# run-house/kubetorch

Measured on NVIDIA H100. Metric: parallel_map_arg_plus_result_GBps, higher is better.
Workload: dtype f32

## Files before the change

kubetorch_b200/csrc/ktb_mlp.cu:

```cuda
#include "ktb_common.cuh"

#include <cuda.h>
#include <algorithm>
#include <atomic>
#include <climits>
#include <cmath>
#include <mutex>

namespace ktb {

constexpr int kMlpBlockM = 128;
constexpr int kMlpBlockK = 64;
constexpr int kMlpWgmmaK = 16;
constexpr int kMlpStages = 4;
constexpr int kMlpConsumers = 256;
constexpr int kMlpThreads = kMlpConsumers + 32;
int g_mlp_chunk_rows = 16896;

__device__ __forceinline__ void tma_load_2d(void* smem_dst, const CUtensorMap* map, int c0, int c1, uint64_t* bar) {
  asm volatile(
      "cp.async.bulk.tensor.2d.shared::cluster.global.mbarrier::complete_tx::bytes [%0], [%1, {%3, %4}], [%2];" ::
          "r"(smem_u32(smem_dst)),
      "l"(map), "r"(smem_u32(bar)), "r"(c0), "r"(c1)
      : "memory");
}
__device__ __forceinline__ void prefetch_tensormap(const CUtensorMap* map) {
  asm volatile("prefetch.tensormap [%0];" ::"l"(map) : "memory");
}
__device__ __forceinline__ void mbar_arrive(uint64_t* bar) {
  asm volatile("mbarrier.arrive.shared::cta.b64 _, [%0];" ::"r"(smem_u32(bar)) : "memory");
}
__device__ __forceinline__ void wgmma_fence() { asm volatile("wgmma.fence.sync.aligned;" ::: "memory"); }
__device__ __forceinline__ void wgmma_commit() { asm volatile("wgmma.commit_group.sync.aligned;" ::: "memory"); }
__device__ __forceinline__ void wgmma_wait_all() { asm volatile("wgmma.wait_group.sync.aligned 0;" ::: "memory"); }

__device__ __forceinline__ uint64_t make_smem_desc_sw128(const void* smem_tile) {
  const uint32_t addr = smem_u32(smem_tile);
  uint64_t d = 0;
  d |= (uint64_t)((addr & 0x3FFFFu) >> 4);
  d |= (uint64_t)1 << 16;
  d |= (uint64_t)(1024u >> 4) << 32;
  d |= (uint64_t)1 << 62;
  return d;
}

template <int N>
struct Wgmma;
template <>
struct Wgmma<256> {
  __device__ __forceinline__ static void mma(float (&d)[128], uint64_t adesc, uint64_t bdesc, uint32_t scale_d) {
    asm volatile(
        "{\n"
        ".reg .pred p;\n"
        "setp.ne.b32 p, %130, 0;\n"
        "wgmma.mma_async.sync.aligned.m64n256k16.f32.bf16.bf16 "
        "{%0,%1,%2,%3,%4,%5,%6,%7,%8,%9,%10,%11,%12,%13,%14,%15,%16,%17,%18,%19,%20,%21,%22,%23,%24,%25,%26,%27,%28,%29,%30,%31,%32,%33,%34,%35,%36,%37,%38,%39,%40,%41,%42,%43,%44,%45,%46,%47,%48,%49,%50,%51,%52,%53,%54,%55,%56,%57,%58,%59,%60,%61,%62,%63,%64,%65,%66,%67,%68,%69,%70,%71,%72,%73,%74,%75,%76,%77,%78,%79,%80,%81,%82,%83,%84,%85,%86,%87,%88,%89,%90,%91,%92,%93,%94,%95,%96,%97,%98,%99,%100,%101,%102,%103,%104,%105,%106,%107,%108,%109,%110,%111,%112,%113,%114,%115,%116,%117,%118,%119,%120,%121,%122,%123,%124,%125,%126,%127}, "
        "%128, %129, p, 1, 1, 0, 0;\n"
        "}\n"
        : "+f"(d[0]), "+f"(d[1]), "+f"(d[2]), "+f"(d[3]), "+f"(d[4]), "+f"(d[5]), "+f"(d[6]), "+f"(d[7]), "+f"(d[8]), "+f"(d[9]), "+f"(d[10]), "+f"(d[11]), "+f"(d[12]), "+f"(d[13]), "+f"(d[14]), "+f"(d[15]), "+f"(d[16]), "+f"(d[17]), "+f"(d[18]), "+f"(d[19]), "+f"(d[20]), "+f"(d[21]), "+f"(d[22]), "+f"(d[23]), "+f"(d[24]), "+f"(d[25]), "+f"(d[26]), "+f"(d[27]), "+f"(d[28]), "+f"(d[29]), "+f"(d[30]), "+f"(d[31]), "+f"(d[32]), "+f"(d[33]), "+f"(d[34]), "+f"(d[35]), "+f"(d[36]), "+f"(d[37]), "+f"(d[38]), "+f"(d[39]), "+f"(d[40]), "+f"(d[41]), "+f"(d[42]), "+f"(d[43]), "+f"(d[44]), "+f"(d[45]), "+f"(d[46]), "+f"(d[47]), "+f"(d[48]), "+f"(d[49]), "+f"(d[50]), "+f"(d[51]), "+f"(d[52]), "+f"(d[53]), "+f"(d[54]), "+f"(d[55]), "+f"(d[56]), "+f"(d[57]), "+f"(d[58]), "+f"(d[59]), "+f"(d[60]), "+f"(d[61]), "+f"(d[62]), "+f"(d[63]), "+f"(d[64]), "+f"(d[65]), "+f"(d[66]), "+f"(d[67]), "+f"(d[68]), "+f"(d[69]), "+f"(d[70]), "+f"(d[71]), "+f"(d[72]), "+f"(d[73]), "+f"(d[74]), "+f"(d[75]), "+f"(d[76]), "+f"(d[77]), "+f"(d[78]), "+f"(d[79]), "+f"(d[80]), "+f"(d[81]), "+f"(d[82]), "+f"(d[83]), "+f"(d[84]), "+f"(d[85]), "+f"(d[86]), "+f"(d[87]), "+f"(d[88]), "+f"(d[89]), "+f"(d[90]), "+f"(d[91]), "+f"(d[92]), "+f"(d[93]), "+f"(d[94]), "+f"(d[95]), "+f"(d[96]), "+f"(d[97]), "+f"(d[98]), "+f"(d[99]), "+f"(d[100]), "+f"(d[101]), "+f"(d[102]), "+f"(d[103]), "+f"(d[104]), "+f"(d[105]), "+f"(d[106]), "+f"(d[107]), "+f"(d[108]), "+f"(d[109]), "+f"(d[110]), "+f"(d[111]), "+f"(d[112]), "+f"(d[113]), "+f"(d[114]), "+f"(d[115]), "+f"(d[116]), "+f"(d[117]), "+f"(d[118]), "+f"(d[119]), "+f"(d[120]), "+f"(d[121]), "+f"(d[122]), "+f"(d[123]), "+f"(d[124]), "+f"(d[125]), "+f"(d[126]), "+f"(d[127])
        : "l"(adesc), "l"(bdesc), "r"(scale_d));
  }
};

template <>
struct Wgmma<128> {
  __device__ __forceinline__ static void mma(float (&d)[64], uint64_t adesc, uint64_t bdesc, uint32_t scale_d) {
    asm volatile(
        "{\n"
        ".reg .pred p;\n"
        "setp.ne.b32 p, %66, 0;\n"
        "wgmma.mma_async.sync.aligned.m64n128k16.f32.bf16.bf16 "
        "{%0,%1,%2,%3,%4,%5,%6,%7,%8,%9,%10,%11,%12,%13,%14,%15,%16,%17,%18,%19,%20,%21,%22,%23,%24,%25,%26,%27,%28,%29,%30,%31,%32,%33,%34,%35,%36,%37,%38,%39,%40,%41,%42,%43,%44,%45,%46,%47,%48,%49,%50,%51,%52,%53,%54,%55,%56,%57,%58,%59,%60,%61,%62,%63}, "
        "%64, %65, p, 1, 1, 0, 0;\n"
        "}\n"
        : "+f"(d[0]), "+f"(d[1]), "+f"(d[2]), "+f"(d[3]), "+f"(d[4]), "+f"(d[5]), "+f"(d[6]), "+f"(d[7]), "+f"(d[8]), "+f"(d[9]), "+f"(d[10]), "+f"(d[11]), "+f"(d[12]), "+f"(d[13]), "+f"(d[14]), "+f"(d[15]), "+f"(d[16]), "+f"(d[17]), "+f"(d[18]), "+f"(d[19]), "+f"(d[20]), "+f"(d[21]), "+f"(d[22]), "+f"(d[23]), "+f"(d[24]), "+f"(d[25]), "+f"(d[26]), "+f"(d[27]), "+f"(d[28]), "+f"(d[29]), "+f"(d[30]), "+f"(d[31]), "+f"(d[32]), "+f"(d[33]), "+f"(d[34]), "+f"(d[35]), "+f"(d[36]), "+f"(d[37]), "+f"(d[38]), "+f"(d[39]), "+f"(d[40]), "+f"(d[41]), "+f"(d[42]), "+f"(d[43]), "+f"(d[44]), "+f"(d[45]), "+f"(d[46]), "+f"(d[47]), "+f"(d[48]), "+f"(d[49]), "+f"(d[50]), "+f"(d[51]), "+f"(d[52]), "+f"(d[53]), "+f"(d[54]), "+f"(d[55]), "+f"(d[56]), "+f"(d[57]), "+f"(d[58]), "+f"(d[59]), "+f"(d[60]), "+f"(d[61]), "+f"(d[62]), "+f"(d[63])
        : "l"(adesc), "l"(bdesc), "r"(scale_d));
  }
};

template <>
struct Wgmma<64> {
  __device__ __forceinline__ static void mma(float (&d)[32], uint64_t adesc, uint64_t bdesc, uint32_t scale_d) {
    asm volatile(
        "{\n"
        ".reg .pred p;\n"
        "setp.ne.b32 p, %34, 0;\n"
        "wgmma.mma_async.sync.aligned.m64n64k16.f32.bf16.bf16 "
        "{%0,%1,%2,%3,%4,%5,%6,%7,%8,%9,%10,%11,%12,%13,%14,%15,%16,%17,%18,%19,%20,%21,%22,%23,%24,%25,%26,%27,%28,%29,%30,%31}, "
        "%32, %33, p, 1, 1, 0, 0;\n"
        "}\n"
        : "+f"(d[0]), "+f"(d[1]), "+f"(d[2]), "+f"(d[3]), "+f"(d[4]), "+f"(d[5]), "+f"(d[6]), "+f"(d[7]), "+f"(d[8]), "+f"(d[9]), "+f"(d[10]), "+f"(d[11]), "+f"(d[12]), "+f"(d[13]), "+f"(d[14]), "+f"(d[15]), "+f"(d[16]), "+f"(d[17]), "+f"(d[18]), "+f"(d[19]), "+f"(d[20]), "+f"(d[21]), "+f"(d[22]), "+f"(d[23]), "+f"(d[24]), "+f"(d[25]), "+f"(d[26]), "+f"(d[27]), "+f"(d[28]), "+f"(d[29]), "+f"(d[30]), "+f"(d[31])
        : "l"(adesc), "l"(bdesc), "r"(scale_d));
  }
};
template <int BLOCK_N, int STAGES>
struct MlpSmem {
  static constexpr int kABytes = kMlpBlockM * kMlpBlockK * 2;
  static constexpr int kBBytes = BLOCK_N * kMlpBlockK * 2;
  static constexpr int kStageBytes = kABytes + kBBytes;
  static constexpr int kBarrierOff = STAGES * kStageBytes;
  static constexpr int kTotal = kBarrierOff + 2 * STAGES * 8 + 1024 ;
};

template <int BLOCK_N, int STAGES>
__device__ __forceinline__ bool mlp_tile_mainloop(const CUtensorMap* map_a, const CUtensorMap* map_b, int K, int m0,
                                                  int n0, float (&acc)[BLOCK_N / 2]) {
  using S = MlpSmem<BLOCK_N, STAGES>;
  extern __shared__ uint8_t smem_raw[];
  uint8_t* smem = reinterpret_cast<uint8_t*>((reinterpret_cast<uintptr_t>(smem_raw) + 1023) & ~(uintptr_t)1023);
  uint64_t* full = reinterpret_cast<uint64_t*>(smem + S::kBarrierOff);
  uint64_t* empty = full + STAGES;

  const int warp = threadIdx.x >> 5;
  const int lane = threadIdx.x & 31;
  const int num_kb = K / kMlpBlockK;

  if (threadIdx.x == 0) {
#pragma unroll
    for (int s = 0; s < STAGES; ++s) {
      mbar_init(&full[s], 1);
      mbar_init(&empty[s], kMlpConsumers);
    }
    fence_barrier_init();
  }
  __syncthreads();

  if (warp == kMlpConsumers / 32) {
    if (lane == 0) {
      prefetch_tensormap(map_a);
      prefetch_tensormap(map_b);
      for (int kb = 0; kb < num_kb; ++kb) {
        const int s = kb % STAGES;
        mbar_wait(&empty[s], ((kb / STAGES) & 1) ^ 1);
        uint8_t* a_dst = smem + (size_t)s * S::kStageBytes;
        mbar_expect_tx(&full[s], S::kStageBytes);
        tma_load_2d(a_dst, map_a, kb * kMlpBlockK, m0, &full[s]);
        tma_load_2d(a_dst + S::kABytes, map_b, kb * kMlpBlockK, n0, &full[s]);
      }
    }
    return false;
  }

  const int wg = warp >> 2;
#pragma unroll
  for (int i = 0; i < BLOCK_N / 2; ++i) acc[i] = 0.f;
  for (int kb = 0; kb < num_kb; ++kb) {
    const int s = kb % STAGES;
    mbar_wait(&full[s], (kb / STAGES) & 1);
    const uint8_t* a_src = smem + (size_t)s * S::kStageBytes + wg * 64 * 128;
    const uint64_t adesc = make_smem_desc_sw128(a_src);
    const uint64_t bdesc = make_smem_desc_sw128(smem + (size_t)s * S::kStageBytes + S::kABytes);
    wgmma_fence();
#pragma unroll
    for (int k = 0; k < kMlpBlockK / kMlpWgmmaK; ++k) {
      Wgmma<BLOCK_N>::mma(acc, adesc + (uint64_t)(2 * k), bdesc + (uint64_t)(2 * k), (uint32_t)((kb | k) != 0));
    }
    wgmma_commit();
    wgmma_wait_all();
    mbar_arrive(&empty[s]);
  }
  return true;
}

__device__ __forceinline__ bool argmax_before(float v, int col, float best, int best_col) {
  const bool v_nan = v != v, best_nan = best != best;
  if (v_nan || best_nan) return v_nan && (!best_nan || col < best_col);
  return v > best || (v == best && col < best_col);
}

__device__ __forceinline__ void layer_pair(float a0, float a1, float a2, float a3, const __nv_bfloat16* bias, int col,
                                           int n_valid, int relu, __nv_bfloat162& y0, __nv_bfloat162& y1) {
  float v[4] = {a0, a1, a2, a3};
  if (bias != nullptr) {
#pragma unroll
    for (int c = 0; c < 2; ++c) {
      if (col + c < n_valid) {
        const float b = __bfloat162float(bias[col + c]);
        v[c] += b;
        v[2 + c] += b;
      }
    }
  }
  if (relu) {
#pragma unroll
    for (int q = 0; q < 4; ++q) v[q] = fmaxf(v[q], 0.f);
  }
  y0 = __floats2bfloat162_rn(v[0], v[1]);
  y1 = __floats2bfloat162_rn(v[2], v[3]);
}

template <int BLOCK_N, int STAGES>
__global__ void __launch_bounds__(kMlpThreads, 1)
    mlp_layer_wgmma_kernel(const __grid_constant__ CUtensorMap map_a, const __grid_constant__ CUtensorMap map_b,
                           const __nv_bfloat16* __restrict__ bias, __nv_bfloat16* __restrict__ C,
                           int64_t* __restrict__ actions, int ldc, int n_valid, int K, int rows, int relu) {
  const int n0 = blockIdx.x * BLOCK_N;
  const int m0 = blockIdx.y * kMlpBlockM;
  const int lane = threadIdx.x & 31;
  const int col0 = n0 + 2 * (lane & 3);
  float acc[BLOCK_N / 2];
  if (!mlp_tile_mainloop<BLOCK_N, STAGES>(&map_a, &map_b, K, m0, n0, acc)) return;
  const int warp = threadIdx.x >> 5;
  const int wg = warp >> 2;

  const int row = m0 + wg * 64 + (warp & 3) * 16 + (lane >> 2);
  const bool st0 = row < rows, st1 = row + 8 < rows;
  const bool pairs = C != nullptr && (ldc & 1) == 0 && ((uintptr_t)C & 3) == 0;
  if (pairs && actions == nullptr && n0 + BLOCK_N <= n_valid) {
    __nv_bfloat16* p0 = C + (size_t)row * ldc + col0;
    __nv_bfloat16* p1 = p0 + (size_t)8 * ldc;
#pragma unroll
    for (int j = 0; j < BLOCK_N / 8; ++j) {
      __nv_bfloat162 y0, y1;
      layer_pair(acc[4 * j], acc[4 * j + 1], acc[4 * j + 2], acc[4 * j + 3], bias, col0 + 8 * j, n_valid, relu, y0, y1);
      if (st0) *reinterpret_cast<__nv_bfloat162*>(p0 + 8 * j) = y0;
      if (st1) *reinterpret_cast<__nv_bfloat162*>(p1 + 8 * j) = y1;
    }
    return;
  }
  float best[2] = {-INFINITY, -INFINITY};
  int best_col[2] = {INT_MAX, INT_MAX};
#pragma unroll
  for (int j = 0; j < BLOCK_N / 8; ++j) {
    const int col = col0 + 8 * j;
    __nv_bfloat162 y0, y1;
    layer_pair(acc[4 * j], acc[4 * j + 1], acc[4 * j + 2], acc[4 * j + 3], bias, col, n_valid, relu, y0, y1);
    if (C != nullptr) {
      __nv_bfloat16* p0 = C + (size_t)row * ldc + col;
      __nv_bfloat16* p1 = p0 + (size_t)8 * ldc;
      if (pairs && col + 1 < n_valid) {
        if (st0) *reinterpret_cast<__nv_bfloat162*>(p0) = y0;
        if (st1) *reinterpret_cast<__nv_bfloat162*>(p1) = y1;
      } else {
        if (st0 && col < n_valid) p0[0] = y0.x;
        if (st1 && col < n_valid) p1[0] = y1.x;
        if (st0 && col + 1 < n_valid) p0[1] = y0.y;
        if (st1 && col + 1 < n_valid) p1[1] = y1.y;
      }
    }
    if (actions != nullptr) {
      const float r[4] = {__low2float(y0), __high2float(y0), __low2float(y1), __high2float(y1)};
#pragma unroll
      for (int q = 0; q < 4; ++q) {
        const int h = q >> 1, c = col + (q & 1);
        if (c < n_valid && argmax_before(r[q], c, best[h], best_col[h])) {
          best[h] = r[q];
          best_col[h] = c;
        }
      }
    }
  }
  if (actions != nullptr) {
#pragma unroll
    for (int h = 0; h < 2; ++h) {
#pragma unroll
      for (int m = 1; m <= 2; m <<= 1) {
        const float ov = __shfl_xor_sync(0xffffffffu, best[h], m);
        const int oc = __shfl_xor_sync(0xffffffffu, best_col[h], m);
        if (argmax_before(ov, oc, best[h], best_col[h])) {
          best[h] = ov;
          best_col[h] = oc;
        }
      }
    }
    if ((lane & 3) == 0) {
      if (st0) actions[row] = best_col[0];
      if (st1) actions[row + 8] = best_col[1];
    }
  }
}

typedef CUresult (*PFN_tensorMapEncodeTiled)(CUtensorMap*, CUtensorMapDataType, cuuint32_t, void*, const cuuint64_t*,
                                             const cuuint64_t*, const cuuint32_t*, const cuuint32_t*,
                                             CUtensorMapInterleave, CUtensorMapSwizzle, CUtensorMapL2promotion,
                                             CUtensorMapFloatOOBfill);
static PFN_tensorMapEncodeTiled g_encode = nullptr;
static std::once_flag g_encode_once;

static int get_encoder() {
  std::call_once(g_encode_once, [] {
    void* fn = nullptr;
    cudaDriverEntryPointQueryResult qres;
    if (cudaGetDriverEntryPoint("cuTensorMapEncodeTiled", &fn, cudaEnableDefault, &qres) == cudaSuccess &&
        qres == cudaDriverEntryPointSuccess)
      g_encode = reinterpret_cast<PFN_tensorMapEncodeTiled>(fn);
  });
  KTB_REQUIRE(g_encode != nullptr, KTB_ERR_CUDA, "cuTensorMapEncodeTiled is not available from the driver");
  return KTB_OK;
}

static int encode_map(CUtensorMap* map, const void* base, uint64_t rows, uint64_t cols, uint32_t box_rows);

static int make_map(CUtensorMap* map, const void* base, uint64_t rows, uint64_t cols, uint32_t box_rows) {
  struct Key {
    const void* base;
    uint64_t rows, cols;
    uint32_t box;
    bool operator==(const Key& o) const { return base == o.base && rows == o.rows && cols == o.cols && box == o.box; }
  };
  struct Slot {
    Key key;
    CUtensorMap map;
    bool used = false;
  };
  constexpr int kSlots = 64;
  thread_local Slot cache[kSlots];
  const Key k{base, rows, cols, box_rows};
  const size_t h = ((uintptr_t)base >> 8) * 0x9E3779B97F4A7C15ull + rows * 31 + cols * 7 + box_rows;
  Slot& s = cache[h % kSlots];
  if (s.used && s.key == k) {
    *map = s.map;
    return KTB_OK;
  }
  int rc = encode_map(map, base, rows, cols, box_rows);
  if (rc) return rc;
  s.key = k;
  s.map = *map;
  s.used = true;
  return KTB_OK;
}

static int encode_map(CUtensorMap* map, const void* base, uint64_t rows, uint64_t cols, uint32_t box_rows) {
  cuuint64_t gdim[2] = {cols, rows};
  cuuint64_t gstride[1] = {cols * 2};
  cuuint32_t box[2] = {(cuuint32_t)kMlpBlockK, box_rows};
  cuuint32_t estr[2] = {1, 1};
  CUresult r = g_encode(map, CU_TENSOR_MAP_DATA_TYPE_BFLOAT16, 2, const_cast<void*>(base), gdim, gstride, box, estr,
                        CU_TENSOR_MAP_INTERLEAVE_NONE, CU_TENSOR_MAP_SWIZZLE_128B, CU_TENSOR_MAP_L2_PROMOTION_L2_256B,
                        CU_TENSOR_MAP_FLOAT_OOB_FILL_NONE);
  KTB_REQUIRE(r == CUDA_SUCCESS, KTB_ERR_CUDA, "cuTensorMapEncodeTiled failed with CUresult %d", (int)r);
  return KTB_OK;
}

template <typename KernelT>
static int ensure_smem_attr(KernelT kfn, int smem_bytes, std::atomic<unsigned>& done_mask, int dev) {
  if (dev >= 0 && dev < 32 && (done_mask.load(std::memory_order_acquire) & (1u << dev))) return KTB_OK;
  cudaError_t e = cudaFuncSetAttribute(kfn, cudaFuncAttributeMaxDynamicSharedMemorySize, smem_bytes);
  if (e != cudaSuccess) {
    set_error("cudaFuncSetAttribute(max dynamic shared memory = %d) failed: %s", smem_bytes, cudaGetErrorString(e));
    return KTB_ERR_CUDA;
  }
  if (dev >= 0 && dev < 32) done_mask.fetch_or(1u << dev, std::memory_order_release);
  return KTB_OK;
}

template <int BLOCK_N>
static int launch_layer(int dev, const void* A, const void* B, const void* bias, void* C, int64_t* actions, size_t M,
                        int N, int K, int ldc, bool relu, cudaStream_t stream) {
  using S = MlpSmem<BLOCK_N, kMlpStages>;
  static_assert(S::kTotal <= 232448, "the TMA ring must fit the 227 KiB a block may own");
  CUtensorMap ma, mb;
  int rc = make_map(&ma, A, M, (uint64_t)K, kMlpBlockM);
  if (rc) return rc;
  rc = make_map(&mb, B, (uint64_t)N, (uint64_t)K, BLOCK_N);
  if (rc) return rc;
  auto kfn = mlp_layer_wgmma_kernel<BLOCK_N, kMlpStages>;
  static std::atomic<unsigned> attr_done{0};
  rc = ensure_smem_attr(kfn, S::kTotal, attr_done, dev);
  if (rc) return rc;
  dim3 grid((unsigned)((N + BLOCK_N - 1) / BLOCK_N), (unsigned)((M + kMlpBlockM - 1) / kMlpBlockM));
  kfn<<<grid, kMlpThreads, S::kTotal, stream>>>(ma, mb, static_cast<const __nv_bfloat16*>(bias),
                                                static_cast<__nv_bfloat16*>(C), actions, ldc, N, K, (int)M, relu);
  KTB_CK(cudaGetLastError());
  return KTB_OK;
}

struct MlpParams {
  const void *W1, *b1, *W2, *b2, *W3, *b3;
  void* logits;
  int64_t* actions;
};

static int mlp_hidden(int dev, const void* A, const void* W, const void* b, void* H, size_t rows, int d_hidden, int K,
                      cudaStream_t st) {
  return launch_layer<256>(dev, A, W, b, H, nullptr, rows, d_hidden, K, d_hidden, true, st);
}

static int mlp_head(int dev, const MlpParams& p, const void* h2, size_t r0, size_t rows, int d_hidden, int d_out,
                    cudaStream_t st) {
  void* y = p.logits ? static_cast<__nv_bfloat16*>(p.logits) + r0 * d_out : nullptr;
  int64_t* act = p.actions ? p.actions + r0 : nullptr;
  if (d_out <= 64) return launch_layer<64>(dev, h2, p.W3, p.b3, y, act, rows, d_out, d_hidden, d_out, false, st);
  if (d_out <= 128) return launch_layer<128>(dev, h2, p.W3, p.b3, y, act, rows, d_out, d_hidden, d_out, false, st);
  return launch_layer<256>(dev, h2, p.W3, p.b3, y, act, rows, d_out, d_hidden, d_out, false, st);
}

static int mlp_check(const char* fn, size_t M, int d_in, int d_hidden, int d_out, const MlpParams& p, const void* obs,
                     const void* scratch, const void* stage) {
  KTB_REQUIRE(d_in > 0 && d_in % kMlpBlockK == 0, KTB_ERR_ARG, "%s: d_in=%d must be a multiple of 64", fn, d_in);
  KTB_REQUIRE(d_hidden > 0 && d_hidden % 256 == 0, KTB_ERR_ARG, "%s: d_hidden=%d must be a multiple of 256", fn,
              d_hidden);
  if (M > 0) {
    KTB_REQUIRE(p.logits || p.actions, KTB_ERR_ARG, "%s: logits and actions are both null", fn);
    KTB_REQUIRE(d_out >= 1, KTB_ERR_ARG, "%s: d_out=%d must be positive", fn, d_out);
    KTB_REQUIRE(d_out <= 256, KTB_ERR_UNSUPPORTED, "%s: d_out=%d (heads up to 256 wide)", fn, d_out);
    KTB_REQUIRE((((uintptr_t)p.logits | (uintptr_t)p.b1 | (uintptr_t)p.b2 | (uintptr_t)p.b3) & 1) == 0, KTB_ERR_ARG,
                "%s: logits and biases must be 2-byte aligned", fn);
    KTB_REQUIRE(((uintptr_t)p.actions & 7) == 0, KTB_ERR_ARG, "%s: actions must be 8-byte aligned", fn);
  }
  KTB_REQUIRE((((uintptr_t)obs | (uintptr_t)p.W1 | (uintptr_t)p.W2 | (uintptr_t)p.W3 | (uintptr_t)scratch |
                (uintptr_t)stage) & 15) == 0,
              KTB_ERR_ARG, "%s: obs, weights, scratch and stage must be 16-byte aligned", fn);
  return KTB_OK;
}
}

using namespace ktb;

extern "C" {

size_t ktb_mlp_scratch_bytes(size_t M, int d_hidden) {
  const size_t rows = std::min<size_t>(M, (size_t)g_mlp_chunk_rows);
  return 2 * rows * (size_t)d_hidden * 2;
}

size_t ktb_mlp_stage_bytes(size_t M, int d_in) {
  const size_t rows = std::min<size_t>(M, (size_t)g_mlp_chunk_rows);
  return 2 * rows * (size_t)d_in * 2;
}

int g_mlp_stage_ce = 0;

static int mlp_run(const char* fn, int dev, const void* obs, size_t M, int d_in, int d_hidden, int d_out,
                   const MlpParams& p, void* scratch, void* stage, uintptr_t stream) {
  int rc = require_device(dev);
  if (rc) return rc;
  if (M == 0) return KTB_OK;
  KTB_REQUIRE(obs && p.W1 && p.W2 && p.W3 && scratch, KTB_ERR_ARG, "%s: null argument", fn);
  rc = mlp_check(fn, M, d_in, d_hidden, d_out, p, obs, scratch, stage);
  if (rc) return rc;
  KTB_REQUIRE(g_mlp_chunk_rows % kMlpBlockM == 0 && g_mlp_chunk_rows > 0, KTB_ERR_ARG, "%s: bad chunk rows", fn);
  rc = get_encoder();
  if (rc) return rc;
  KTB_GUARD(dev);
  DeviceInfo* di = device_info(dev);
  cudaStream_t st = reinterpret_cast<cudaStream_t>(stream);
  cudaStream_t side = di->stream_exec;
  const size_t chunk = std::min<size_t>(M, (size_t)g_mlp_chunk_rows);
  __nv_bfloat16* h1 = static_cast<__nv_bfloat16*>(scratch);
  __nv_bfloat16* h2 = h1 + chunk * (size_t)d_hidden;
  const __nv_bfloat16* x = static_cast<const __nv_bfloat16*>(obs);
  __nv_bfloat16* stg = static_cast<__nv_bfloat16*>(stage);
  const MapParams ident = make_params(1, 0);
  cudaEvent_t evs[5] = {nullptr, nullptr, nullptr, nullptr, nullptr};
  struct EvGuard {
    cudaEvent_t* e;
    ~EvGuard() {
      for (int i = 0; i < 5; ++i)
        if (e[i]) cudaEventDestroy(e[i]);
    }
  } ev_guard{evs};
  static std::mutex side_mu[kMaxDevices];
  std::unique_lock<std::mutex> side_lock;
  if (stg) {
    side_lock = std::unique_lock<std::mutex>(side_mu[dev]);
    for (int i = 0; i < 5; ++i) KTB_CK(cudaEventCreateWithFlags(&evs[i], cudaEventDisableTiming));
    KTB_CK(cudaEventRecord(evs[0], st));
    KTB_CK(cudaStreamWaitEvent(side, evs[0], 0));
  }
  size_t c = 0;
  for (size_t r0 = 0; r0 < M; r0 += chunk, ++c) {
    const size_t rows = std::min(chunk, M - r0);
    const __nv_bfloat16* a1 = x + r0 * d_in;
    if (stg) {
      const int b = (int)(c & 1);
      __nv_bfloat16* dstb = stg + (size_t)b * chunk * d_in;
      if (c >= 2) KTB_CK(cudaStreamWaitEvent(side, evs[3 + b], 0));
      if (g_mlp_stage_ce) {
        KTB_CK(cudaMemcpyAsync(dstb, a1, rows * (size_t)d_in * 2, cudaMemcpyDefault, side));
      } else {
        rc = launch_map(dev, KTB_OP_IDENTITY, KTB_U8, a1, dstb, rows * (size_t)d_in * 2, ident, KTB_VARIANT_AUTO, side);
        if (rc) return rc;
      }
      KTB_CK(cudaEventRecord(evs[1 + b], side));
      KTB_CK(cudaStreamWaitEvent(st, evs[1 + b], 0));
      a1 = dstb;
    }
    rc = mlp_hidden(dev, a1, p.W1, p.b1, h1, rows, d_hidden, d_in, st);
    if (rc) return rc;
    if (stg) KTB_CK(cudaEventRecord(evs[3 + (int)(c & 1)], st));
    rc = mlp_hidden(dev, h1, p.W2, p.b2, h2, rows, d_hidden, d_hidden, st);
    if (rc) return rc;
    rc = mlp_head(dev, p, h2, r0, rows, d_hidden, d_out, st);
    if (rc) return rc;
  }
  return KTB_OK;
}

namespace ktb {
__global__ void mlp_wait_ready_kernel(const unsigned long long* ready, unsigned long long seq, unsigned int* status) {
  if (threadIdx.x == 0) (void)spin_until(ready, seq, status);
}
__global__ void mlp_ack_kernel(unsigned long long* ack, unsigned long long seq) {
  if (threadIdx.x == 0) {
    __threadfence_system();
    st_release_sys(ack, seq);
  }
}
}

static int mlp_pushed_run(const char* fn, int dev, const void* stage_local, size_t stage_stride, size_t M, int d_in,
                          int d_hidden, int d_out, const MlpParams& p, void* scratch, void* ctrl_local,
                          void* ctrl_root_peer, int rank, size_t chunk_rows, unsigned long long seq, uintptr_t stream) {
  int rc = require_device(dev);
  if (rc) return rc;
  KTB_REQUIRE(stage_local && ctrl_local && ctrl_root_peer && p.W1 && p.W2 && p.W3 && scratch, KTB_ERR_ARG,
              "%s: null argument", fn);
  KTB_REQUIRE(rank >= 0 && rank < 16 && seq > 0, KTB_ERR_ARG, "%s: bad rank/seq", fn);
  KTB_REQUIRE(M % kMlpBlockM == 0, KTB_ERR_ARG, "%s: M=%zu must be a multiple of %d", fn, M, kMlpBlockM);
  KTB_REQUIRE(chunk_rows > 0 && chunk_rows % kMlpBlockM == 0, KTB_ERR_ARG,
              "%s: chunk_rows=%zu must be a positive multiple of %d", fn, chunk_rows, kMlpBlockM);
  rc = mlp_check(fn, M, d_in, d_hidden, d_out, p, stage_local, scratch, nullptr);
  if (rc) return rc;
  const size_t n_chunks = (M + chunk_rows - 1) / chunk_rows;
  KTB_REQUIRE(n_chunks <= KTB_PUSH_MAX_CHUNKS, KTB_ERR_ARG, "%s: %zu chunks exceed %d", fn, n_chunks,
              KTB_PUSH_MAX_CHUNKS);
  KTB_REQUIRE(M * (size_t)d_in * 2 <= stage_stride, KTB_ERR_ARG, "%s: shard exceeds stage_stride", fn);
  rc = get_encoder();
  if (rc) return rc;
  KTB_GUARD(dev);
  cudaStream_t st = reinterpret_cast<cudaStream_t>(stream);
  uint8_t* cl = static_cast<uint8_t*>(ctrl_local);
  const unsigned long long* ready = reinterpret_cast<const unsigned long long*>(cl + KTB_CTRL_READY);
  unsigned int* status = reinterpret_cast<unsigned int*>(cl + KTB_CTRL_STATUS);
  unsigned long long* ack =
      reinterpret_cast<unsigned long long*>(static_cast<uint8_t*>(ctrl_root_peer) + KTB_CTRL_ACK) + rank;
  const __nv_bfloat16* x =
      reinterpret_cast<const __nv_bfloat16*>(static_cast<const uint8_t*>(stage_local) + (size_t)(seq & 1) * stage_stride);
  __nv_bfloat16* h1 = static_cast<__nv_bfloat16*>(scratch);
  __nv_bfloat16* h2 = h1 + std::min(chunk_rows, M) * (size_t)d_hidden;
  size_t c = 0;
  for (size_t r0 = 0; r0 < M; r0 += chunk_rows, ++c) {
    const size_t rows = std::min(chunk_rows, M - r0);
    mlp_wait_ready_kernel<<<1, 32, 0, st>>>(ready + c, seq, status);
    KTB_CK(cudaGetLastError());
    const __nv_bfloat16* a1 = x + r0 * d_in;
    rc = mlp_hidden(dev, a1, p.W1, p.b1, h1, rows, d_hidden, d_in, st);
    if (rc) return rc;
    rc = mlp_hidden(dev, h1, p.W2, p.b2, h2, rows, d_hidden, d_hidden, st);
    if (rc) return rc;
    rc = mlp_head(dev, p, h2, r0, rows, d_hidden, d_out, st);
    if (rc) return rc;
  }
  mlp_ack_kernel<<<1, 32, 0, st>>>(ack, seq);
  KTB_CK(cudaGetLastError());
  return KTB_OK;
}

int ktb_mlp_bf16_pushed(int dev, const void* stage_local, size_t stage_stride, size_t M, int d_in, int d_hidden, int d_out,
                        const void* W1, const void* W2, const void* W3, void* logits, void* scratch, void* ctrl_local,
                        void* ctrl_root_peer, int rank, size_t chunk_rows, unsigned long long seq, uintptr_t stream) {
  const char* fn = "ktb_mlp_bf16_pushed";
  int rc = require_device(dev);
  if (rc) return rc;
  KTB_REQUIRE(logits || M == 0, KTB_ERR_ARG, "%s: null argument", fn);
  KTB_REQUIRE(d_out == 64, KTB_ERR_UNSUPPORTED, "%s: d_out=%d (the 64-wide head)", fn, d_out);
  const MlpParams p{W1, nullptr, W2, nullptr, W3, nullptr, logits, nullptr};
  return mlp_pushed_run(fn, dev, stage_local, stage_stride, M, d_in, d_hidden, d_out, p, scratch, ctrl_local,
                        ctrl_root_peer, rank, chunk_rows, seq, stream);
}

int ktb_mlp_bf16_policy_pushed(int dev, const void* stage_local, size_t stage_stride, size_t M, int d_in, int d_hidden,
                               int d_out, const void* W1, const void* b1, const void* W2, const void* b2,
                               const void* W3, const void* b3, void* logits, int64_t* actions, void* scratch,
                               void* ctrl_local, void* ctrl_root_peer, int rank, size_t chunk_rows,
                               unsigned long long seq, uintptr_t stream) {
  const MlpParams p{W1, b1, W2, b2, W3, b3, logits, actions};
  return mlp_pushed_run("ktb_mlp_bf16_policy_pushed", dev, stage_local, stage_stride, M, d_in, d_hidden, d_out, p,
                        scratch, ctrl_local, ctrl_root_peer, rank, chunk_rows, seq, stream);
}

static int mlp_run_64(const char* fn, int dev, const void* obs, size_t M, int d_in, int d_hidden, int d_out,
                      const void* W1, const void* W2, const void* W3, void* logits, void* scratch, void* stage,
                      uintptr_t stream) {
  int rc = require_device(dev);
  if (rc || M == 0) return rc;
  KTB_REQUIRE(logits, KTB_ERR_ARG, "%s: null argument", fn);
  KTB_REQUIRE(d_out == 64, KTB_ERR_UNSUPPORTED, "%s: d_out=%d (the 64-wide head)", fn, d_out);
  KTB_REQUIRE(((uintptr_t)logits & 15) == 0, KTB_ERR_ARG, "%s: logits must be 16-byte aligned", fn);
  const MlpParams p{W1, nullptr, W2, nullptr, W3, nullptr, logits, nullptr};
  return mlp_run(fn, dev, obs, M, d_in, d_hidden, d_out, p, scratch, stage, stream);
}

int ktb_mlp_bf16(int dev, const void* obs, size_t M, int d_in, int d_hidden, int d_out, const void* W1,
                 const void* W2, const void* W3, void* logits, void* scratch, uintptr_t stream) {
  return mlp_run_64("ktb_mlp_bf16", dev, obs, M, d_in, d_hidden, d_out, W1, W2, W3, logits, scratch, nullptr, stream);
}

int ktb_mlp_bf16_staged(int dev, const void* obs_peer, size_t M, int d_in, int d_hidden, int d_out, const void* W1,
                        const void* W2, const void* W3, void* logits, void* scratch, void* stage, uintptr_t stream) {
  KTB_REQUIRE(stage, KTB_ERR_ARG, "ktb_mlp_bf16_staged: null stage buffer");
  return mlp_run_64("ktb_mlp_bf16_staged", dev, obs_peer, M, d_in, d_hidden, d_out, W1, W2, W3, logits, scratch, stage,
                    stream);
}

int ktb_mlp_bf16_policy(int dev, const void* obs, size_t M, int d_in, int d_hidden, int d_out, const void* W1,
                        const void* b1, const void* W2, const void* b2, const void* W3, const void* b3, void* logits,
                        int64_t* actions, void* scratch, void* stage, uintptr_t stream) {
  const MlpParams p{W1, b1, W2, b2, W3, b3, logits, actions};
  return mlp_run("ktb_mlp_bf16_policy", dev, obs, M, d_in, d_hidden, d_out, p, scratch, stage, stream);
}

}
```

Measured before the change: 2942.

## Make MLP layer kernel persistent with 2-CTA cluster B multicast and TMA stores

Turns the per-tile MLP GEMM kernel into a persistent kernel over cluster work units, with 2-CTA clusters along M sharing B tiles through TMA multicast. It keeps one wgmma group in flight so stage release overlaps the next MMA, and adds a TMA-store epilogue through swizzled shared memory for hidden layers. The aims are to cut redundant weight loads, launch and tail overhead, and scattered global stores, at the cost of cluster synchronisation, extra shared memory and more complex barrier accounting.

```diff
diff --git a/kubetorch_b200/csrc/ktb_mlp.cu b/kubetorch_b200/csrc/ktb_mlp.cu
--- a/kubetorch_b200/csrc/ktb_mlp.cu
+++ b/kubetorch_b200/csrc/ktb_mlp.cu
@@ -15,6 +15,7 @@
 constexpr int kMlpStages = 4;
 constexpr int kMlpConsumers = 256;
 constexpr int kMlpThreads = kMlpConsumers + 32;
+constexpr int kMlpClusterM = 2;
 int g_mlp_chunk_rows = 16896;
 
 __device__ __forceinline__ void tma_load_2d(void* smem_dst, const CUtensorMap* map, int c0, int c1, uint64_t* bar) {
@@ -32,7 +33,8 @@
 }
 __device__ __forceinline__ void wgmma_fence() { asm volatile("wgmma.fence.sync.aligned;" ::: "memory"); }
 __device__ __forceinline__ void wgmma_commit() { asm volatile("wgmma.commit_group.sync.aligned;" ::: "memory"); }
-__device__ __forceinline__ void wgmma_wait_all() { asm volatile("wgmma.wait_group.sync.aligned 0;" ::: "memory"); }
+template <int N>
+__device__ __forceinline__ void wgmma_wait() { asm volatile("wgmma.wait_group.sync.aligned %0;" ::"n"(N) : "memory"); }
 
 __device__ __forceinline__ uint64_t make_smem_desc_sw128(const void* smem_tile) {
   const uint32_t addr = smem_u32(smem_tile);
@@ -93,74 +95,67 @@
         : "l"(adesc), "l"(bdesc), "r"(scale_d));
   }
 };
+__device__ __forceinline__ uint32_t cluster_ctarank() {
+  uint32_t r;
+  asm volatile("mov.u32 %0, %%cluster_ctarank;" : "=r"(r));
+  return r;
+}
+__device__ __forceinline__ uint32_t cluster_id_x() {
+  uint32_t r;
+  asm volatile("mov.u32 %0, %%clusterid.x;" : "=r"(r));
+  return r;
+}
+__device__ __forceinline__ uint32_t cluster_count_x() {
+  uint32_t r;
+  asm volatile("mov.u32 %0, %%nclusterid.x;" : "=r"(r));
+  return r;
+}
+__device__ __forceinline__ void cluster_sync() {
+  asm volatile("barrier.cluster.arrive.release;\nbarrier.cluster.wait.acquire;" ::: "memory");
+}
+__device__ __forceinline__ void mbar_arrive_cluster(uint64_t* bar, uint32_t rank) {
+  asm volatile(
+      "{\n"
+      ".reg .b32 ra;\n"
+      "mapa.shared::cluster.u32 ra, %0, %1;\n"
+      "mbarrier.arrive.shared::cluster.b64 _, [ra];\n"
+      "}\n" ::"r"(smem_u32(bar)),
+      "r"(rank)
+      : "memory");
+}
+__device__ __forceinline__ void tma_load_2d_multicast(void* smem_dst, const CUtensorMap* map, int c0, int c1,
+                                                      uint64_t* bar, uint16_t mask) {
+  asm volatile(
+      "cp.async.bulk.tensor.2d.shared::cluster.global.mbarrier::complete_tx::bytes.multicast::cluster "
+      "[%0], [%1, {%3, %4}], [%2], %5;" ::"r"(smem_u32(smem_dst)),
+      "l"(map), "r"(smem_u32(bar)), "r"(c0), "r"(c1), "h"(mask)
+      : "memory");
+}
+
 template <int BLOCK_N, int STAGES>
 struct MlpSmem {
   static constexpr int kABytes = kMlpBlockM * kMlpBlockK * 2;
   static constexpr int kBBytes = BLOCK_N * kMlpBlockK * 2;
+  static constexpr int kBPartRows = BLOCK_N / kMlpClusterM;
+  static constexpr int kBPartBytes = kBBytes / kMlpClusterM;
   static constexpr int kStageBytes = kABytes + kBBytes;
-  static constexpr int kBarrierOff = STAGES * kStageBytes;
+  static constexpr int kOutCols = BLOCK_N < 128 ? BLOCK_N : 128;
+  static constexpr int kOutBytes = 64 * kOutCols * 2;
+  static constexpr int kOutOff = STAGES * kStageBytes;
+  static constexpr int kBarrierOff = kOutOff + (kMlpConsumers / 128) * kOutBytes;
   static constexpr int kTotal = kBarrierOff + 2 * STAGES * 8 + 1024 ;
+  static_assert(kBPartRows % 8 == 0, "each multicast part of B must be whole 8-row swizzle atoms");
 };
 
-template <int BLOCK_N, int STAGES>
-__device__ __forceinline__ bool mlp_tile_mainloop(const CUtensorMap* map_a, const CUtensorMap* map_b, int K, int m0,
-                                                  int n0, float (&acc)[BLOCK_N / 2]) {
-  using S = MlpSmem<BLOCK_N, STAGES>;
-  extern __shared__ uint8_t smem_raw[];
-  uint8_t* smem = reinterpret_cast<uint8_t*>((reinterpret_cast<uintptr_t>(smem_raw) + 1023) & ~(uintptr_t)1023);
-  uint64_t* full = reinterpret_cast<uint64_t*>(smem + S::kBarrierOff);
-  uint64_t* empty = full + STAGES;
-
-  const int warp = threadIdx.x >> 5;
-  const int lane = threadIdx.x & 31;
-  const int num_kb = K / kMlpBlockK;
-
-  if (threadIdx.x == 0) {
-#pragma unroll
-    for (int s = 0; s < STAGES; ++s) {
-      mbar_init(&full[s], 1);
-      mbar_init(&empty[s], kMlpConsumers);
-    }
-    fence_barrier_init();
-  }
-  __syncthreads();
-
-  if (warp == kMlpConsumers / 32) {
-    if (lane == 0) {
-      prefetch_tensormap(map_a);
-      prefetch_tensormap(map_b);
-      for (int kb = 0; kb < num_kb; ++kb) {
-        const int s = kb % STAGES;
-        mbar_wait(&empty[s], ((kb / STAGES) & 1) ^ 1);
-        uint8_t* a_dst = smem + (size_t)s * S::kStageBytes;
-        mbar_expect_tx(&full[s], S::kStageBytes);
-        tma_load_2d(a_dst, map_a, kb * kMlpBlockK, m0, &full[s]);
-        tma_load_2d(a_dst + S::kABytes, map_b, kb * kMlpBlockK, n0, &full[s]);
-      }
-    }
-    return false;
-  }
-
-  const int wg = warp >> 2;
-#pragma unroll
-  for (int i = 0; i < BLOCK_N / 2; ++i) acc[i] = 0.f;
-  for (int kb = 0; kb < num_kb; ++kb) {
-    const int s = kb % STAGES;
-    mbar_wait(&full[s], (kb / STAGES) & 1);
-    const uint8_t* a_src = smem + (size_t)s * S::kStageBytes + wg * 64 * 128;
-    const uint64_t adesc = make_smem_desc_sw128(a_src);
-    const uint64_t bdesc = make_smem_desc_sw128(smem + (size_t)s * S::kStageBytes + S::kABytes);
-    wgmma_fence();
-#pragma unroll
-    for (int k = 0; k < kMlpBlockK / kMlpWgmmaK; ++k) {
-      Wgmma<BLOCK_N>::mma(acc, adesc + (uint64_t)(2 * k), bdesc + (uint64_t)(2 * k), (uint32_t)((kb | k) != 0));
-    }
-    wgmma_commit();
-    wgmma_wait_all();
-    mbar_arrive(&empty[s]);
-  }
-  return true;
-}
+struct MlpSchedule {
+  int m_blocks, n_tiles, units;
+  __host__ __device__ MlpSchedule(int rows, int n_valid, int block_n)
+      : m_blocks((rows + kMlpBlockM - 1) / kMlpBlockM),
+        n_tiles((n_valid + block_n - 1) / block_n),
+        units((m_blocks + kMlpClusterM - 1) / kMlpClusterM * n_tiles) {}
+  __device__ int m_block(int unit, int rank) const { return unit / n_tiles * kMlpClusterM + rank; }
+  __device__ int n_tile(int unit) const { return unit % n_tiles; }
+};
 
 __device__ __forceinline__ bool argmax_before(float v, int col, float best, int best_col) {
   const bool v_nan = v != v, best_nan = best != best;
@@ -189,20 +184,14 @@
   y1 = __floats2bfloat162_rn(v[2], v[3]);
 }
 
-template <int BLOCK_N, int STAGES>
-__global__ void __launch_bounds__(kMlpThreads, 1)
-    mlp_layer_wgmma_kernel(const __grid_constant__ CUtensorMap map_a, const __grid_constant__ CUtensorMap map_b,
-                           const __nv_bfloat16* __restrict__ bias, __nv_bfloat16* __restrict__ C,
-                           int64_t* __restrict__ actions, int ldc, int n_valid, int K, int rows, int relu) {
-  const int n0 = blockIdx.x * BLOCK_N;
-  const int m0 = blockIdx.y * kMlpBlockM;
+template <int BLOCK_N>
+__device__ __forceinline__ void mlp_tile_epilogue(const float (&acc)[BLOCK_N / 2], const __nv_bfloat16* __restrict__ bias,
+                                                  __nv_bfloat16* __restrict__ C, int64_t* __restrict__ actions, int ldc,
+                                                  int n_valid, int rows, int relu, int m0, int n0) {
+  const int warp = threadIdx.x >> 5;
   const int lane = threadIdx.x & 31;
+  const int wg = warp >> 2;
   const int col0 = n0 + 2 * (lane & 3);
-  float acc[BLOCK_N / 2];
-  if (!mlp_tile_mainloop<BLOCK_N, STAGES>(&map_a, &map_b, K, m0, n0, acc)) return;
-  const int warp = threadIdx.x >> 5;
-  const int wg = warp >> 2;
-
   const int row = m0 + wg * 64 + (warp & 3) * 16 + (lane >> 2);
   const bool st0 = row < rows, st1 = row + 8 < rows;
   const bool pairs = C != nullptr && (ldc & 1) == 0 && ((uintptr_t)C & 3) == 0;
@@ -268,6 +257,140 @@
       if (st1) actions[row + 8] = best_col[1];
     }
   }
+}
+
+__device__ __forceinline__ void tma_store_2d(const CUtensorMap* map, const void* smem_src, int c0, int c1) {
+  asm volatile("cp.async.bulk.tensor.2d.global.shared::cta.bulk_group [%0, {%2, %3}], [%1];" ::"l"(map),
+               "r"(smem_u32(smem_src)), "r"(c0), "r"(c1)
+               : "memory");
+}
+__device__ __forceinline__ void named_barrier_sync(int id, int threads) {
+  asm volatile("bar.sync %0, %1;" ::"r"(id), "r"(threads) : "memory");
+}
+
+template <int BLOCK_N, int STAGES>
+__device__ __forceinline__ void mlp_tile_epilogue_tma(const float (&acc)[BLOCK_N / 2],
+                                                      const __nv_bfloat16* __restrict__ bias, const CUtensorMap* map_c,
+                                                      uint8_t* out, int n_valid, int relu, int m0, int n0) {
+  using S = MlpSmem<BLOCK_N, STAGES>;
+  const int warp = threadIdx.x >> 5;
+  const int lane = threadIdx.x & 31;
+  const int wg = warp >> 2;
+  const bool leader = (threadIdx.x & 127) == 0;
+  const int r = (warp & 3) * 16 + (lane >> 2);
+  const int col0 = n0 + 2 * (lane & 3);
+#pragma unroll
+  for (int pass = 0; pass < BLOCK_N / S::kOutCols; ++pass) {
+    if (leader) bulk_wait_read<0>();
+    named_barrier_sync(1 + wg, 128);
+#pragma unroll
+    for (int jj = 0; jj < S::kOutCols / 8; ++jj) {
+      const int j = pass * (S::kOutCols / 8) + jj;
+      __nv_bfloat162 y0, y1;
+      layer_pair(acc[4 * j], acc[4 * j + 1], acc[4 * j + 2], acc[4 * j + 3], bias, col0 + 8 * j, n_valid, relu, y0, y1);
+      uint8_t* p = out + (jj / 8) * (64 * 128) + r * 128 + (((jj & 7) ^ (r & 7)) << 4) + 4 * (lane & 3);
+      *reinterpret_cast<__nv_bfloat162*>(p) = y0;
+      *reinterpret_cast<__nv_bfloat162*>(p + 8 * 128) = y1;
+    }
+    fence_proxy_async_smem();
+    named_barrier_sync(1 + wg, 128);
+    if (leader) {
+#pragma unroll
+      for (int b = 0; b < S::kOutCols / 64; ++b)
+        tma_store_2d(map_c, out + b * (64 * 128), n0 + pass * S::kOutCols + b * 64, m0 + wg * 64);
+      bulk_commit();
+    }
+  }
+}
+
+template <int BLOCK_N, int STAGES>
+__global__ void __launch_bounds__(kMlpThreads, 1)
+    mlp_layer_wgmma_kernel(const __grid_constant__ CUtensorMap map_a, const __grid_constant__ CUtensorMap map_b,
+                           const __grid_constant__ CUtensorMap map_c, const __nv_bfloat16* __restrict__ bias,
+                           __nv_bfloat16* __restrict__ C, int64_t* __restrict__ actions, int ldc, int n_valid, int K,
+                           int rows, int relu, int tma_store) {
+  using S = MlpSmem<BLOCK_N, STAGES>;
+  extern __shared__ uint8_t smem_raw[];
+  uint8_t* smem = reinterpret_cast<uint8_t*>((reinterpret_cast<uintptr_t>(smem_raw) + 1023) & ~(uintptr_t)1023);
+  uint64_t* full = reinterpret_cast<uint64_t*>(smem + S::kBarrierOff);
+  uint64_t* empty = full + STAGES;
+
+  const int warp = threadIdx.x >> 5;
+  const int lane = threadIdx.x & 31;
+  const int num_kb = K / kMlpBlockK;
+  const uint32_t rank = cluster_ctarank();
+  const int first_unit = (int)cluster_id_x(), unit_step = (int)cluster_count_x();
+  const MlpSchedule sched(rows, n_valid, BLOCK_N);
+
+  if (threadIdx.x == 0) {
+#pragma unroll
+    for (int s = 0; s < STAGES; ++s) {
+      mbar_init(&full[s], 1);
+      mbar_init(&empty[s], kMlpClusterM * (kMlpConsumers / 128));
+    }
+    fence_barrier_init();
+  }
+  cluster_sync();
+
+  if (warp == kMlpConsumers / 32) {
+    if (lane == 0) {
+      prefetch_tensormap(&map_a);
+      prefetch_tensormap(&map_b);
+      const uint16_t mask = (uint16_t)((1u << kMlpClusterM) - 1);
+      uint32_t it = 0;
+      for (int u = first_unit; u < sched.units; u += unit_step) {
+        const int m0 = min(sched.m_block(u, rank), sched.m_blocks - 1) * kMlpBlockM;
+        const int b_row = min(sched.n_tile(u) * BLOCK_N + (int)rank * S::kBPartRows, n_valid - 1);
+        for (int kb = 0; kb < num_kb; ++kb, ++it) {
+          const uint32_t s = it % STAGES;
+          mbar_wait(&empty[s], ((it / STAGES) & 1) ^ 1);
+          uint8_t* a_dst = smem + (size_t)s * S::kStageBytes;
+          mbar_expect_tx(&full[s], S::kStageBytes);
+          tma_load_2d(a_dst, &map_a, kb * kMlpBlockK, m0, &full[s]);
+          tma_load_2d_multicast(a_dst + S::kABytes + rank * S::kBPartBytes, &map_b, kb * kMlpBlockK, b_row, &full[s],
+                                mask);
+        }
+      }
+    }
+  } else {
+    const int wg = warp >> 2;
+    const bool releaser = lane == 0 && (warp & 3) < kMlpClusterM;
+    const uint32_t release_rank = (uint32_t)(warp & 3);
+    uint32_t it = 0;
+    for (int u = first_unit; u < sched.units; u += unit_step) {
+      float acc[BLOCK_N / 2];
+#pragma unroll
+      for (int i = 0; i < BLOCK_N / 2; ++i) acc[i] = 0.f;
+      for (int kb = 0; kb < num_kb; ++kb, ++it) {
+        const uint32_t s = it % STAGES;
+        mbar_wait(&full[s], (it / STAGES) & 1);
+        const uint8_t* a_src = smem + (size_t)s * S::kStageBytes + wg * 64 * 128;
+        const uint64_t adesc = make_smem_desc_sw128(a_src);
+        const uint64_t bdesc = make_smem_desc_sw128(smem + (size_t)s * S::kStageBytes + S::kABytes);
+        wgmma_fence();
+#pragma unroll
+        for (int k = 0; k < kMlpBlockK / kMlpWgmmaK; ++k) {
+          Wgmma<BLOCK_N>::mma(acc, adesc + (uint64_t)(2 * k), bdesc + (uint64_t)(2 * k), (uint32_t)((kb | k) != 0));
+        }
+        wgmma_commit();
+        if (kb > 0) {
+          wgmma_wait<1>();
+          if (releaser) mbar_arrive_cluster(&empty[(it - 1) % STAGES], release_rank);
+        }
+      }
+      wgmma_wait<0>();
+      if (releaser) mbar_arrive_cluster(&empty[(it - 1) % STAGES], release_rank);
+      const int m0 = sched.m_block(u, rank) * kMlpBlockM, n0 = sched.n_tile(u) * BLOCK_N;
+      if (!tma_store) {
+        mlp_tile_epilogue<BLOCK_N>(acc, bias, C, actions, ldc, n_valid, rows, relu, m0, n0);
+      } else if (m0 + wg * 64 < rows) {
+        mlp_tile_epilogue_tma<BLOCK_N, STAGES>(acc, bias, &map_c, smem + S::kOutOff + wg * S::kOutBytes, n_valid,
+                                               relu, m0, n0);
+      }
+    }
+    if (tma_store && (threadIdx.x & 127) == 0) bulk_wait_all<0>();
+  }
+  cluster_sync();
 }
 
 typedef CUresult (*PFN_tensorMapEncodeTiled)(CUtensorMap*, CUtensorMapDataType, cuuint32_t, void*, const cuuint64_t*,
@@ -346,22 +469,48 @@
 
 template <int BLOCK_N>
 static int launch_layer(int dev, const void* A, const void* B, const void* bias, void* C, int64_t* actions, size_t M,
-                        int N, int K, int ldc, bool relu, cudaStream_t stream) {
+                        int N, int K, int ldc, bool relu, bool local_c, cudaStream_t stream) {
   using S = MlpSmem<BLOCK_N, kMlpStages>;
   static_assert(S::kTotal <= 232448, "the TMA ring must fit the 227 KiB a block may own");
-  CUtensorMap ma, mb;
+  CUtensorMap ma, mb, mc;
   int rc = make_map(&ma, A, M, (uint64_t)K, kMlpBlockM);
   if (rc) return rc;
-  rc = make_map(&mb, B, (uint64_t)N, (uint64_t)K, BLOCK_N);
-  if (rc) return rc;
+  rc = make_map(&mb, B, (uint64_t)N, (uint64_t)K, S::kBPartRows);
+  if (rc) return rc;
+  const bool tma_store = local_c && C != nullptr && actions == nullptr && N % BLOCK_N == 0 && ldc == N &&
+                         ((uintptr_t)C & 15) == 0;
+  mc = ma;
+  if (tma_store) {
+    rc = make_map(&mc, C, M, (uint64_t)N, 64);
+    if (rc) return rc;
+  }
   auto kfn = mlp_layer_wgmma_kernel<BLOCK_N, kMlpStages>;
   static std::atomic<unsigned> attr_done{0};
   rc = ensure_smem_attr(kfn, S::kTotal, attr_done, dev);
   if (rc) return rc;
-  dim3 grid((unsigned)((N + BLOCK_N - 1) / BLOCK_N), (unsigned)((M + kMlpBlockM - 1) / kMlpBlockM));
-  kfn<<<grid, kMlpThreads, S::kTotal, stream>>>(ma, mb, static_cast<const __nv_bfloat16*>(bias),
-                                                static_cast<__nv_bfloat16*>(C), actions, ldc, N, K, (int)M, relu);
-  KTB_CK(cudaGetLastError());
+  cudaLaunchConfig_t cfg = {};
+  cudaLaunchAttribute attr[1];
+  attr[0].id = cudaLaunchAttributeClusterDimension;
+  attr[0].val.clusterDim.x = kMlpClusterM;
+  attr[0].val.clusterDim.y = 1;
+  attr[0].val.clusterDim.z = 1;
+  cfg.blockDim = dim3(kMlpThreads);
+  cfg.dynamicSmemBytes = S::kTotal;
+  cfg.stream = stream;
+  cfg.attrs = attr;
+  cfg.numAttrs = 1;
+  static std::atomic<int> resident[kMaxDevices];
+  int clusters = dev >= 0 && dev < kMaxDevices ? resident[dev].load(std::memory_order_relaxed) : 0;
+  if (clusters == 0) {
+    cfg.gridDim = dim3(kMlpClusterM);
+    KTB_CK(cudaOccupancyMaxActiveClusters(&clusters, kfn, &cfg));
+    KTB_REQUIRE(clusters > 0, KTB_ERR_CUDA, "no cluster of %d MLP layer CTAs fits on device %d", kMlpClusterM, dev);
+    if (dev >= 0 && dev < kMaxDevices) resident[dev].store(clusters, std::memory_order_relaxed);
+  }
+  const MlpSchedule sched((int)M, N, BLOCK_N);
+  cfg.gridDim = dim3((unsigned)(std::min(sched.units, clusters) * kMlpClusterM));
+  KTB_CK(cudaLaunchKernelEx(&cfg, kfn, ma, mb, mc, static_cast<const __nv_bfloat16*>(bias),
+                            static_cast<__nv_bfloat16*>(C), actions, ldc, N, K, (int)M, (int)relu, (int)tma_store));
   return KTB_OK;
 }
 
@@ -373,16 +522,16 @@
 
 static int mlp_hidden(int dev, const void* A, const void* W, const void* b, void* H, size_t rows, int d_hidden, int K,
                       cudaStream_t st) {
-  return launch_layer<256>(dev, A, W, b, H, nullptr, rows, d_hidden, K, d_hidden, true, st);
+  return launch_layer<256>(dev, A, W, b, H, nullptr, rows, d_hidden, K, d_hidden, true, true, st);
 }
 
 static int mlp_head(int dev, const MlpParams& p, const void* h2, size_t r0, size_t rows, int d_hidden, int d_out,
                     cudaStream_t st) {
   void* y = p.logits ? static_cast<__nv_bfloat16*>(p.logits) + r0 * d_out : nullptr;
   int64_t* act = p.actions ? p.actions + r0 : nullptr;
-  if (d_out <= 64) return launch_layer<64>(dev, h2, p.W3, p.b3, y, act, rows, d_out, d_hidden, d_out, false, st);
-  if (d_out <= 128) return launch_layer<128>(dev, h2, p.W3, p.b3, y, act, rows, d_out, d_hidden, d_out, false, st);
-  return launch_layer<256>(dev, h2, p.W3, p.b3, y, act, rows, d_out, d_hidden, d_out, false, st);
+  if (d_out <= 64) return launch_layer<64>(dev, h2, p.W3, p.b3, y, act, rows, d_out, d_hidden, d_out, false, false, st);
+  if (d_out <= 128) return launch_layer<128>(dev, h2, p.W3, p.b3, y, act, rows, d_out, d_hidden, d_out, false, false, st);
+  return launch_layer<256>(dev, h2, p.W3, p.b3, y, act, rows, d_out, d_hidden, d_out, false, false, st);
 }
 
 static int mlp_check(const char* fn, size_t M, int d_in, int d_hidden, int d_out, const MlpParams& p, const void* obs,
```

After: 2940 (median of 6 runs). About the same (-0.1%).
